# intelligent-environments-lab/CityLearn

Hardware: AMD Instinct MI355X
Metric: building-timesteps/sec at 17 bldgs x 65536 envs; HBM GB/s vs roofline (higher is better)
Workload: dtype f32 (battery soc chain in f64); 1 GPU; citylearn_challenge_2022_phase_all tables (17 buildings, the full year, 8 760 h) x 65536 envs per GPU, cl_step_f32 mode A (one env step per launch, state in HBM, fresh uniform random actions from an 8-tensor ring), env batch sharded over GPUs, no collective; CLD_F64_CHAIN: battery soc chain in float64, degraded capacity carried as the capacity loss; envs_per_gpu=65536, buildings=17, env_pitch=65536, precision=CLD_F64_CHAIN (StepEngine default): 1e-4 free-running over whole episodes, launch=hipGraph replay, reward=RewardFunction, reps=1, statistic=median of reps (each: MAX over ranks)

## Files before the change

### citylearn_amd/csrc/cl_kernels.hip

```cpp
#include "cl_trace.h"
#include "cl_unit.h"
#include "cl_plan.h"
#ifndef CL_LEAN_NT_LOADS
#define CL_LEAN_NT_LOADS true
#endif
#include "cl_philox.h"

#include <type_traits>
#include <mutex>
#include <stdarg.h>
#include <string.h>
#include <stdio.h>

namespace {

int hip_fail(hipError_t e, const char* what) {
    return fail(CL_EHIP, "%s: %s", what, hipGetErrorString(e));
}

hipError_t ensure_dynamic_lds(const void* fn, size_t bytes) {
    struct Seen { const void* fn; int dev; size_t bytes; };
    static Seen seen[64];
    static int n_seen = 0;
    static std::mutex mu;
    int dev = 0;
    if (hipError_t e = hipGetDevice(&dev); e != hipSuccess) return e;
    std::lock_guard<std::mutex> lock(mu);
    for (int i = 0; i < n_seen; ++i)
        if (seen[i].fn == fn && seen[i].dev == dev && seen[i].bytes >= bytes) return hipSuccess;
    if (hipError_t e = hipFuncSetAttribute(fn, hipFuncAttributeMaxDynamicSharedMemorySize, (int)bytes); e != hipSuccess) return e;
    for (int i = 0; i < n_seen; ++i)
        if (seen[i].fn == fn && seen[i].dev == dev) { seen[i].bytes = bytes; return hipSuccess; }
    if (n_seen < 64) seen[n_seen++] = {fn, dev, bytes};
    return hipSuccess;
}

struct StepArgs {
// ... 51 lines not shown
            for (int i = 0; i < VEC; ++i) dst[i] = v[i];
        }
    } else vload<VEC>(dst, p);
}

template <int VEC>
CL_DEV void vstore(float* __restrict__ p, const float (&src)[VEC]) {
    using V = typename Vec<VEC>::type;
    V v;
    if constexpr (VEC == 1) v = src[0];
    else {
#pragma unroll
        for (int i = 0; i < VEC; ++i) v[i] = src[i];
    }
    *reinterpret_cast<V*>(p) = v;
}

template <int VEC, bool NT>
CL_DEV void pstore(float* __restrict__ p, const float (&src)[VEC]) {
    using V = typename Vec<VEC>::type;
    V v;
    if constexpr (VEC == 1) v = src[0];
    else {
#pragma unroll
        for (int i = 0; i < VEC; ++i) v[i] = src[i];
    }
    if constexpr (NT) __builtin_nontemporal_store(v, reinterpret_cast<V*>(p));
    else *reinterpret_cast<V*>(p) = v;
}
struct NtOn { static constexpr bool value = true; };
struct NtOff { static constexpr bool value = false; };

template <int VEC>
CL_DEV void load_action(float (&dst)[VEC], const StepArgs& a, int col, int env0) {
    if (col < 0) {
#pragma unroll
        for (int i = 0; i < VEC; ++i) dst[i] = 0.0f;
        return;
    }
    const float* p = a.actions + (long long)col * a.act_stride_col;
    if (a.act_stride_env == 1) vload<VEC>(dst, p + env0);
    else {
#pragma unroll
        for (int i = 0; i < VEC; ++i) dst[i] = p[(long long)(env0 + i) * a.act_stride_env];
    }
}

#include "cl_flex.h"

constexpr int NQ = CL_NQ;

struct KpiSeries { float prev, ramp, dsum, dmax, msum, mmax, amax; };
CL_DEV void kpi_series_fetch(KpiSeries& s, const float* __restrict__ k, long long n_env);
CL_DEV void kpi_series_apply(float* __restrict__ k, long long n_env, int t, float v, const KpiSeries& s);
CL_DEV void kpi_series_update(float* __restrict__ k, long long n_env, int t, float v);

CL_DEV int fold_shift(int opw) { return opw <= 16 ? 4 : opw <= 32 ? 5 : 6; }
template <int TILE>
CL_DEV float fold_prefetch(const StepArgs& a, int w, int lane, long long plane, int bx, int by) {
    if (a.fused_finish != 2) return 0.0f;
    const int opw = (NQ * TILE + a.n_chunks - 1) / a.n_chunks;
    const int sh = fold_shift(opw);
    const int i = w * 64 + lane, chunk = i >> sh, j = i & ((1 << sh) - 1), o = by * opw + j;
    const int e = bx * TILE + o % TILE;
    if (chunk < a.n_chunks && j < opw && o < NQ * TILE && e < a.n_env)
        return a.out_bldg[(long long)CLO_RESERVED * plane + ((long long)((a.t + 1) & 1) * a.n_chunks + chunk) * NQ * a.n_env + (long long)(o / TILE) * a.n_env + e];
    return 0.0f;
}
CL_DEV void fold_stash(const StepArgs& a, float* lds_fold, int w, int lane, float v) {
    if (a.fused_finish == 2 && w < 16) lds_fold[w * 64 + lane] = v;
}
template <int TILE>
CL_DEV void fold_finish(const StepArgs& a, const float* lds_fold, int w, int lane, int bx, int by) {
    const int opw = (NQ * TILE + a.n_chunks - 1) / a.n_chunks;
    const int sh = fold_shift(opw);
    const int k = lane & 15;
    for (int j = w; j < opw; j += 16) {
        const int o = by * opw + j;
        if (o >= NQ * TILE || bx * TILE + o % TILE >= a.n_env) continue;
// ... 416 lines not shown
                const float rw = cl::unit_reward<false>(rkind, B, S, O.net);
                o_soc[i] = S.soc; o_eff[i] = S.eff; o_deg[i] = S.degcap; o_net[i] = O.net; o_rw[i] = rw;
                q_net[i] += O.net; q_cost[i] += O.cost; q_em[i] += O.emission;
                q_rw[i] += marl_partial ? cl::marl_reward(O.net, 1.0f) : rw;
            }
            if constexpr (FOLD) {
                if (!folded && b + a.nw >= b_hi) { fold_stash(a, lds_fold, w, lane, fold_prev); folded = true; }
            }
            if (b + a.nw < b_hi) fetch(cur, b + a.nw);
            if (batt) {
                pstore<VEC, NT>(a.state + CLS_B_SOC * plane + off, o_soc);
                pstore<VEC, NT>(a.state + CLS_B_EFF * plane + off, o_eff);
                pstore<VEC, NT>(a.state + CLS_B_DEGCAP * plane + off, o_deg);
            }
            pstore<VEC, NT>(a.out_bldg + CLO_NET * plane + off, o_net);
            if (rkind != CLR_MARL) pstore<VEC, NT>(a.out_bldg + CLO_REWARD * plane + off, o_rw);
        }
    }
    if constexpr (FOLD) {
        if (!folded) fold_stash(a, lds_fold, w, lane, fold_prev);
    }
    district_reduce<VEC, false, FOLD>(a, lds, w, lane, env0, live, plane, rkind, q_net, q_cost, q_em, q_rw, a.nw, lds_fold);
}

struct ObsFusedArgs {
    float* __restrict__ obs;
    const float* __restrict__ table;
    int n_cols, pitch, row;
    short start[CL_OBS_FUSED_BLDG + 1];
    cl_obs_dep deps[CLOB_MAX_DEPS];
    int lean_ok;
};

template <int VEC, bool FLEX, bool NT, bool OBS, bool KPI = false, int PREC = 0>
CL_DEV void lean_step_body(const StepArgs& a, float* lds, const ObsFusedArgs* of) {
    constexpr bool F64 = PREC == 1;
    constexpr int TILE = 64 * VEC;
    const int lane = threadIdx.x & 63;
    const int w = __builtin_amdgcn_readfirstlane(threadIdx.x >> 6);
    const int env0 = blockIdx.x * TILE + lane * VEC;
    const bool live = env0 < a.n_env;
    const long long plane = (long long)a.n_bldg * a.ld;
    const int rkind = (a.flags & CLD_REWARD_MASK) >> CLD_REWARD_SHIFT;
    const bool quirk = a.flags & CLD_REF_T0_QUIRK;
    const bool act_by_bldg = (a.flags & CLD_ES_COL_IS_BLDG) && a.act_stride_env == 1;
    const int ts_row = a.t + (a.env_row0 ? a.env_row0[(blockIdx.x * TILE) / CL_ROW0_BLOCK] : 0);
    const int bb[2] = {w, w + a.nw};
    const bool own[2] = {bb[0] < a.n_bldg, bb[1] < a.n_bldg};

    float q_net[VEC], q_cost[VEC], q_em[VEC], q_rw[VEC];
#pragma unroll
    for (int i = 0; i < VEC; ++i) q_net[i] = q_cost[i] = q_em[i] = q_rw[i] = 0.0f;
    float s_soc[2][VEC], s_eff[2][VEC], s_deg[2][VEC], a_es[2][VEC];
    [[maybe_unused]] float s_efl[2][VEC], s_dgl[2][VEC];
    constexpr bool NTL = NT && CL_LEAN_NT_LOADS && (KPI || FLEX || VEC == 2);
    CL_TRACE_DECL;
    CL_TRACE_ENTRY(0);
    CL_TRACE_CYCLES_ENTRY(4);
    if (live) {
#pragma unroll
        for (int m = 0; m < 2; ++m) {
            if (!own[m]) continue;
            const long long off = (long long)bb[m] * a.ld + env0;
            pload<VEC, NTL>(s_soc[m], a.state + CLS_B_SOC * plane + off);
            pload<VEC, NTL>(s_eff[m], a.state + CLS_B_EFF * plane + off);
            pload<VEC, NTL>(s_deg[m], a.state + CLS_B_DEGCAP * plane + off);
            if constexpr (F64) {
                pload<VEC, NTL>(s_efl[m], a.state + CLS_B_EFF_LO * plane + off);
                pload<VEC, NTL>(s_dgl[m], a.state + CLS_B_DEGCAP_LO * plane + off);
            }
            if (act_by_bldg) pload<VEC, NTL>(a_es[m], a.actions + (long long)bb[m] * a.act_stride_col + env0);
        }
    }
#pragma unroll
    for (int m = 0; m < 2; ++m) {
        if (!own[m]) continue;
        const int b = bb[m];
        cl::Bp B;
        cl::load_bp<false>(B, a.params + (long long)b * CL_NP);
        cl::Row R;
        cl::load_row<false>(R, a.ts + ((long long)ts_row * a.n_bldg + b) * CL_NF, B.flags);
        [[maybe_unused]] int od_n = 0, od_col[CL_OBS_FUSED_PER_BLDG], od_src[CL_OBS_FUSED_PER_BLDG];
        [[maybe_unused]] float od_scale[CL_OBS_FUSED_PER_BLDG], od_base[CL_OBS_FUSED_PER_BLDG];
        if constexpr (OBS) {
            const float* __restrict__ trow = of->table + (size_t)(of->row + (ts_row - a.t)) * of->n_cols;
            const int d0 = of->start[b];
            od_n = of->start[b + 1] - d0;
#pragma unroll
            for (int k = 0; k < CL_OBS_FUSED_PER_BLDG; ++k) {
                const int d = min(d0 + min(k, max(od_n - 1, 0)), CLOB_MAX_DEPS - 1);
                od_col[k] = of->deps[d].col; od_src[k] = of->deps[d].src; od_scale[k] = of->deps[d].scale;
                od_base[k] = trow[od_col[k]];
            }
        }
        if (!live) continue;
        const long long off = (long long)b * a.ld + env0;
        const bool batt = B.flags & CLF_BATTERY;
        if (!act_by_bldg) load_action<VEC>(a_es[m], a, B.a_es, env0);
        CL_TRACE_WAITV(1 + 4 * m, s_deg[m][0]);
        float o_net[VEC], o_rw[VEC];
        [[maybe_unused]] float o_cb[VEC];
        const int fbi = (FLEX && (B.flags & CLF_FLEX)) ? (int)B.p[CLP_FLEX_INDEX] : -1;
        float x_load[VEC];
        if (FLEX && fbi >= 0) vload<VEC>(x_load, a.flex_out + (long long)CLX_LOAD * a.n_flex_bldg * a.n_env + (long long)fbi * a.n_env + env0);
        if constexpr (FLEX) {
#pragma unroll
            for (int i = 0; i < VEC; ++i) {
                cl::State S;
                S.soc = batt ? s_soc[m][i] : 0.0f; S.eff = batt ? s_eff[m][i] : 1.0f; S.degcap = batt ? s_deg[m][i] : 0.0f;
                S.cs = S.hs = S.ds = 0.0f;
                const cl::Act act = {0.0f, 0.0f, 0.0f, B.a_es >= 0 ? a_es[m][i] : 0.0f, 0.0f, 0.0f};
                cl::Out O;
                cl::unit_step<false>(B, R, a.t, quirk, act, S, O);
                if (FLEX && fbi >= 0) cl::apply_flex(false, R.price, R.carbon, x_load[i], 0.0f, O);
                const float rw = cl::unit_reward<false>(rkind, B, S, O.net);
                s_soc[m][i] = S.soc; s_eff[m][i] = S.eff; s_deg[m][i] = S.degcap;
                o_net[i] = O.net; o_rw[i] = rw;
                q_net[i] += O.net; q_cost[i] += O.cost; q_em[i] += O.emission;
                q_rw[i] += (FLEX && rkind == CLR_EV) ? cl::marl_reward(O.net, 1.0f) : rw;
            }
        } else {
            const bool first = quirk && a.t == 0;
            float c_ns = first ? 3.0f * R.nsl : R.nsl;
            float sol = R.sol;
            const float cbk = first ? 2.0f : 1.0f;
            CL_PIN_V(c_ns); CL_PIN_V(sol);
            float soc_rw[VEC];
            if (F64 && batt) {
                if constexpr (F64) {
                    cl::BattP64 B64;
                    cl::load_batt64(B64, B.p);
                    if (B.a_es < 0) {
#pragma unroll
                        for (int i = 0; i < VEC; ++i) a_es[m][i] = 0.0f;
                    }
#pragma unroll
                    for (int i = 0; i < VEC; ++i) {
                        cl::State S = {s_soc[m][i], s_eff[m][i], s_deg[m][i], 0.0f, 0.0f, 0.0f, s_efl[m][i], s_dgl[m][i]};
                        const float eb = cl::battery_charge_ref(B64, (double)a_es[m][i] * B64.pow * B64.dt / B64.r, a.t == 0, S);
                        s_soc[m][i] = S.soc; s_eff[m][i] = S.eff; s_deg[m][i] = S.degcap; s_efl[m][i] = S.eff_lo; s_dgl[m][i] = S.deg_lo;
                        soc_rw[i] = S.soc;
                        o_cb[i] = cbk * eb;
                        o_net[i] = fmaf(c_ns + o_cb[i], B.r, sol);
                    }
                }
            } else if (PREC == 2 && batt) {
                if constexpr (PREC == 2) {
                    cl::BattC bc;
                    cl::load_battc(bc, B.p);
                    if (B.a_es < 0) {
#pragma unroll
                        for (int i = 0; i < VEC; ++i) a_es[m][i] = 0.0f;
                    }
#pragma unroll
                    for (int i = 0; i < VEC; ++i) {
                        cl::State S = {s_soc[m][i], s_eff[m][i], s_deg[m][i], 0.0f, 0.0f, 0.0f};
                        const float eb = cl::battery_charge_chain(bc, a_es[m][i], INFINITY, S);
                        s_soc[m][i] = S.soc; s_eff[m][i] = S.eff; s_deg[m][i] = S.degcap;
                        soc_rw[i] = S.soc;
                        o_cb[i] = cbk * eb;
                        o_net[i] = fmaf(c_ns + o_cb[i], B.r, sol);
                    }
                }
            } else if (batt) {
                cl::BattP Bv = B.batt;
                CL_PIN_V(Bv.cpc_a0); CL_PIN_V(Bv.cpc_b0); CL_PIN_V(Bv.cpc_a1); CL_PIN_V(Bv.cpc_b1);
                CL_PIN_V(Bv.pec_a0); CL_PIN_V(Bv.pec_b0); CL_PIN_V(Bv.pec_a1); CL_PIN_V(Bv.pec_b1);
                CL_PIN_V(Bv.pec_a2); CL_PIN_V(Bv.pec_b2); CL_PIN_V(Bv.pec_a3); CL_PIN_V(Bv.pec_b3);
                if (B.a_es < 0) {
#pragma unroll
                    for (int i = 0; i < VEC; ++i) a_es[m][i] = 0.0f;
                }
#pragma unroll
                for (int i = 0; i < VEC; ++i) {
                    cl::State S = {s_soc[m][i], s_eff[m][i], s_deg[m][i], 0.0f, 0.0f, 0.0f};
                    const float eb = cl::battery_energy(Bv, a_es[m][i] * Bv.pdt, S);
                    s_soc[m][i] = S.soc; s_eff[m][i] = S.eff; s_deg[m][i] = S.degcap;
                    soc_rw[i] = S.soc;
                    o_cb[i] = cbk * eb;
                    o_net[i] = fmaf(c_ns + o_cb[i], B.r, sol);
                }
            } else {
#pragma unroll
                for (int i = 0; i < VEC; ++i) { o_net[i] = fmaf(c_ns + 0.0f, B.r, sol); soc_rw[i] = 0.0f; o_cb[i] = 0.0f; }
            }
            cl::lean_rewards<VEC>(rkind, B, soc_rw, o_net, o_rw);
#pragma unroll
            for (int i = 0; i < VEC; ++i) {
                q_net[i] += o_net[i]; q_cost[i] += cl::mul_rn(o_net[i], R.price); q_em[i] += fmaxf(0.0f, o_net[i] * R.carbon);
                q_rw[i] += o_rw[i];
            }
        }
        CL_TRACE_AFTER(2 + 4 * m, o_rw[VEC - 1]);
        if (batt) {
            pstore<VEC, NT>(a.state + CLS_B_SOC * plane + off, s_soc[m]);
            pstore<VEC, NT>(a.state + CLS_B_EFF * plane + off, s_eff[m]);
            pstore<VEC, NT>(a.state + CLS_B_DEGCAP * plane + off, s_deg[m]);
            if constexpr (F64) {
                pstore<VEC, NT>(a.state + CLS_B_EFF_LO * plane + off, s_efl[m]);
                pstore<VEC, NT>(a.state + CLS_B_DEGCAP_LO * plane + off, s_dgl[m]);
            }
        }
        pstore<VEC, NT>(a.out_bldg + CLO_NET * plane + off, o_net);
        if (rkind != CLR_MARL && !(FLEX && rkind == CLR_EV)) pstore<VEC, NT>(a.out_bldg + CLO_REWARD * plane + off, o_rw);
        if constexpr (KPI && !FLEX) {
            float k_pos[VEC], k_net[VEC], k_em[VEC], k_cost[VEC];
            float* kp = a.kpi_bldg + off;
            vload<VEC>(k_pos, kp + (long long)CLK_C_POS * plane); vload<VEC>(k_net, kp + (long long)CLK_C_NET * plane);
            vload<VEC>(k_em, kp + (long long)CLK_C_EMISSION * plane); vload<VEC>(k_cost, kp + (long long)CLK_C_COST * plane);
            const bool block_sums = lane == 0 && (blockIdx.x * TILE) % CL_ROW0_BLOCK == 0;
            float b_pos = 0.0f, b_net = 0.0f, b_em = 0.0f, b_cost = 0.0f, b_exp = 0.0f;
            if (block_sums) {
                b_pos = kp[(long long)CLK_B_POS * plane]; b_net = kp[(long long)CLK_B_NET * plane];
                b_em = kp[(long long)CLK_B_EMISSION * plane]; b_cost = kp[(long long)CLK_B_COST * plane];
                b_exp = kp[(long long)CLK_EXPECTED_ALL * plane];
            }
#pragma unroll
            for (int i = 0; i < VEC; ++i) {
                k_pos[i] += fmaxf(o_net[i], 0.0f); k_net[i] += o_net[i];
                k_em[i] += fmaxf(o_net[i] * R.carbon, 0.0f); k_cost[i] += fmaxf(o_net[i] * R.price, 0.0f);
            }
            pstore<VEC, NT>(kp + (long long)CLK_C_POS * plane, k_pos); pstore<VEC, NT>(kp + (long long)CLK_C_NET * plane, k_net);
            pstore<VEC, NT>(kp + (long long)CLK_C_EMISSION * plane, k_em); pstore<VEC, NT>(kp + (long long)CLK_C_COST * plane, k_cost);
            const float c_ns0 = (quirk && a.t == 0) ? 3.0f * R.nsl : R.nsl;
            const float base = fmaf(c_ns0, B.r, R.sol);
            if (lane == 0) lds[(size_t)a.nw * NQ * TILE + b] = base;
            if (block_sums) {
                kp[(long long)CLK_B_POS * plane] = b_pos + fmaxf(base, 0.0f);
                kp[(long long)CLK_B_NET * plane] = b_net + base;
                kp[(long long)CLK_B_EMISSION * plane] = b_em + fmaxf(base * R.carbon, 0.0f);
                kp[(long long)CLK_B_COST * plane] = b_cost + fmaxf(base * R.price, 0.0f);
                kp[(long long)CLK_EXPECTED_ALL * plane] = b_exp + R.nsl;
            }
        }
        if constexpr (OBS) {
            float* tile = lds + (size_t)a.nw * NQ * TILE;
#pragma unroll
            for (int k = 0; k < CL_OBS_FUSED_PER_BLDG; ++k) {
                if (k >= od_n) break;
                const int col = od_col[k], src = od_src[k];
                const float scale = od_scale[k], base = od_base[k];
                const bool is_out = (src >> 28) == CLOB_KIND_OUT;
                const int pl = (src >> 20) & 0xFF;
#pragma unroll
                for (int i = 0; i < VEC; ++i) {
                    const float v = is_out ? (pl == CLO_NET ? o_net[i] : o_rw[i])
                                           : (pl == CLS_B_SOC ? s_soc[m][i] : pl == CLS_B_EFF ? s_eff[m][i] : s_deg[m][i]);
                    tile[(size_t)(lane * VEC + i) * of->pitch + col] = fmaf(v, scale, base);
                }
            }
        }
        CL_TRACE_AFTER(3 + 4 * m, q_rw[0]);
    }
    if constexpr (OBS) {
        if (w == 0) {
            float* tile = lds + (size_t)a.nw * NQ * TILE;
            for (int c = of->n_cols; c < of->pitch; ++c) {
#pragma unroll
                for (int i = 0; i < VEC; ++i) tile[(size_t)(lane * VEC + i) * of->pitch + c] = 0.0f;
            }
        }
    }
    CL_TRACE_AFTER(13, q_net[0]);
    [[maybe_unused]] KpiSeries base_pre;
    [[maybe_unused]] const bool base_writer = KPI && !FLEX && threadIdx.x == blockDim.x - 1 && (blockIdx.x * TILE) % CL_ROW0_BLOCK == 0;
    if constexpr (KPI && !FLEX) {
        if (base_writer) kpi_series_fetch(base_pre, a.kpi_env + (long long)CLKE_PER_COND * a.n_env + blockIdx.x * TILE, a.n_env);
    }
    district_reduce<VEC, FLEX, false, KPI && !FLEX>(a, lds, w, lane, env0, live, plane, rkind, q_net, q_cost, q_em, q_rw, a.nw);
    if constexpr (KPI && !FLEX) {
        if (base_writer) {
            float sum = 0.0f;
            for (int b = 0; b < a.n_bldg; ++b) sum += lds[(size_t)a.nw * NQ * TILE + b];
            kpi_series_apply(a.kpi_env + (long long)CLKE_PER_COND * a.n_env + blockIdx.x * TILE, a.n_env, a.t, sum, base_pre);
        }
    }
    if constexpr (OBS) {
        typedef float f4 __attribute__((ext_vector_type(4)));
        const int tile_env0 = blockIdx.x * TILE;
        const int rows = min(TILE, a.n_env - tile_env0);
        const f4* src4 = reinterpret_cast<const f4*>(lds + (size_t)a.nw * NQ * TILE);
        f4* dst4 = reinterpret_cast<f4*>(of->obs + (size_t)tile_env0 * of->pitch);
        const int total4 = rows * of->pitch / 4;
        for (int q = threadIdx.x; q < total4; q += blockDim.x) {
            if constexpr (NT) __builtin_nontemporal_store(src4[q], dst4 + q);
            else dst4[q] = src4[q];
        }
    }
    CL_TRACE_FLUSH();
}

template <int VEC, bool FLEX, bool NT>
__global__ void __launch_bounds__(1024) cl_step_lean_kernel(const StepArgs a) {
    extern __shared__ __attribute__((aligned(16))) float lds[];
    lean_step_body<VEC, FLEX, NT, false>(a, lds, nullptr);
}

template <int VEC, bool NT>
__global__ void __launch_bounds__(1024) cl_step_lean_f64_kernel(const StepArgs a) {
    extern __shared__ __attribute__((aligned(16))) float lds[];
    lean_step_body<VEC, false, NT, false, false, 1>(a, lds, nullptr);
}

template <int VEC, bool NT>
__global__ void __launch_bounds__(1024) cl_step_lean_chain_kernel(const StepArgs a) {
    extern __shared__ __attribute__((aligned(16))) float lds[];
    lean_step_body<VEC, false, NT, false, false, 2>(a, lds, nullptr);
}

template <int VEC, bool NT>
__global__ void __launch_bounds__(1024) cl_step_lean_kpi_chain_kernel(const StepArgs a) {
    extern __shared__ __attribute__((aligned(16))) float lds[];
    lean_step_body<VEC, false, NT, false, true, 2>(a, lds, nullptr);
}

template <int VEC, bool NT>
__global__ void __launch_bounds__(1024) cl_step_lean_obs_chain_kernel(const StepArgs a, const ObsFusedArgs of) {
    extern __shared__ __attribute__((aligned(16))) float lds[];
    lean_step_body<VEC, false, NT, true, false, 2>(a, lds, &of);
}

template <int VEC, bool NT>
__global__ void __launch_bounds__(1024) cl_step_lean_kpi_kernel(const StepArgs a) {
    extern __shared__ __attribute__((aligned(16))) float lds[];
    lean_step_body<VEC, false, NT, false, true>(a, lds, nullptr);
}

template <int VEC, bool NT>
__global__ void __launch_bounds__(1024) cl_step_lean_obs_kernel(const StepArgs a, const ObsFusedArgs of) {
    extern __shared__ __attribute__((aligned(16))) float lds[];
    lean_step_body<VEC, false, NT, true>(a, lds, &of);
}

template <int NB, bool NT, int VEC = 1, int PREC = 0>
__global__ void __launch_bounds__(256 / VEC) cl_step_envmajor_kernel(const StepArgs a) {
    constexpr int THREADS = 256 / VEC, TILE = 256;
    const int env = blockIdx.x * TILE + threadIdx.x * VEC;
    const bool live = env < a.n_env;
    const long long plane = (long long)a.n_bldg * a.ld;
    const int rkind = (a.flags & CLD_REWARD_MASK) >> CLD_REWARD_SHIFT;
// ... 1126 lines not shown
```

### citylearn_amd/abi.py

```python
from __future__ import annotations

import re
from pathlib import Path

HEADER = Path(__file__).resolve().parent.parent / 'include' / 'citylearn_amd.h'


def _strip_comments(text: str) -> str:
    text = re.sub(r'/\*.*?\*/', ' ', text, flags=re.S)
    return re.sub(r'//[^\n]*', ' ', text)


def _parse(text: str) -> dict:
    text = _strip_comments(text)
    out: dict = {}
    for m in re.finditer(r'#define\s+(CL\w+)\s+(.+)', text):
        name, expr = m.group(1), m.group(2).strip()
        expr = re.sub(r'(0x[0-9a-fA-F]+|\d+)[uU]\b', r'\1', expr)
        try:
            out[name] = int(eval(expr, {'__builtins__': {}}, out))
        except Exception:
            pass
    for m in re.finditer(r'enum\s+(\w+)\s*\{(.*?)\}', text, flags=re.S):
        nxt = 0
        for item in m.group(2).split(','):
            item = item.strip()
            if not item:
                continue
            if '=' in item:
                name, val = [s.strip() for s in item.split('=')]
                nxt = int(eval(val, {'__builtins__': {}}, out))
            else:
                name = item
            out[name] = nxt
            nxt += 1
    return out


_C = _parse(HEADER.read_text())
globals().update(_C)
CONSTANTS = dict(_C)

EXPORTED_SYMBOLS = sorted(set(re.findall(r'\b(cl_\w+)\s*\(', _strip_comments(HEADER.read_text()))))

assert _C['CLP_USED'] <= _C['CLP_F_FIRST'] and _C['CLP_F_LAST'] < _C['CLP_D_FIRST'] and _C['CLP_D_LAST'] < _C['CL_NP'], 'cl_param overflows CL_NP'
assert _C['CLPD_USED'] * 2 <= _C['CLP_D_LAST'] - _C['CLP_D_FIRST'] + 1 and _C['CLP_D_FIRST'] % 2 == 0 and _C['CL_NP'] % 2 == 0
assert _C['CLP_D_LAST'] < _C['CLP_C_FIRST'] and _C['CLP_C_LAST'] < _C['CL_NP'] and _C['CLP_C_FIRST'] % 2 == 0 and _C['CLPC_USED'] * 2 <= _C['CLP_C_LAST'] - _C['CLP_C_FIRST'] + 1
```

### citylearn_amd/csrc/cl_unit.h

```cpp
#pragma once

#include <stdint.h>
#include "../../include/citylearn_amd.h"

#ifdef CL_HOST_SHIM
#include <math.h>
#include <string.h>
#define CL_DEV inline
namespace cl {
inline float rcp(float x) { return 1.0f / x; }
inline float rsq(float x) { return 1.0f / sqrtf(x); }
inline float fsqrt(float x) { return sqrtf(x); }
inline float med3(float a, float b, float c) { return fmaxf(fminf(a, b), fminf(fmaxf(a, b), c)); }
inline float __uint_as_float(uint32_t u) { float f; memcpy(&f, &u, 4); return f; }
inline float __powf(float a, float b) { return powf(a, b); }
}
#else
#include <hip/hip_runtime.h>
#define CL_DEV __device__ __forceinline__
namespace cl {
CL_DEV float rcp(float x) { return __builtin_amdgcn_rcpf(x); }
CL_DEV float rsq(float x) { return __builtin_amdgcn_rsqf(x); }
CL_DEV float fsqrt(float x) { return __builtin_amdgcn_sqrtf(x); }
CL_DEV float med3(float a, float b, float c) { return __builtin_amdgcn_fmed3f(a, b, c); }
// ... 496 lines not shown
}

template <int N>
CL_DEV void lean_rewards(int kind, const Bp& B, const float (&soc)[N], const float (&net)[N], float (&rw)[N]) {
    switch (kind) {
    case CLR_INDEPENDENT_SAC:
#pragma unroll
        for (int i = 0; i < N; ++i) rw[i] = fminf(-net[i], 0.0f);
        break;
    case CLR_SOLAR_PENALTY: {
        const bool has = pw(B.p, CLP_L_CAP) > CL_ZDP;
#pragma unroll
        for (int i = 0; i < N; ++i) {
            const float sg = net[i] > 0.0f ? 1.0f : (net[i] < 0.0f ? -1.0f : 0.0f), an = fabsf(net[i]);
            rw[i] = has ? -(1.0f + sg * soc[i]) * an : 0.0f;
        }
        break;
    }
    case CLR_MARL: case CLR_EV:
#pragma unroll
        for (int i = 0; i < N; ++i) rw[i] = net[i];
        break;
    default:
        if (B.rw_exponent == 1.0f) {
#pragma unroll
            for (int i = 0; i < N; ++i) rw[i] = -fmaxf(net[i], 0.0f);
        } else {
#pragma unroll
            for (int i = 0; i < N; ++i) rw[i] = -__powf(fmaxf(net[i], 0.0f), B.rw_exponent);
        }
    }
}

CL_DEV float marl_reward(float net, float district_net) {
    const float sg = net < 0.0f ? 1.0f : (net > 0.0f ? -1.0f : 0.0f);
    return sg * 0.01f * net * net * fmaxf(0.0f, district_net);
}

}
```

### citylearn_amd/schema.py

```python
from __future__ import annotations

import hashlib
import json
import math
import os
from dataclasses import dataclass, field
from pathlib import Path
from typing import Any, Dict, List, Mapping, Optional, Sequence, Tuple, Union

import numpy as np

from . import abi

ZERO_DIVISION_PLACEHOLDER = 1e-6
TOLERANCE = 1e-4
DEFAULT_COMFORT_BAND = 2.0

_STORAGE_ACTIONS = ('cooling_storage', 'heating_storage', 'dhw_storage', 'electrical_storage')
_DEVICE_ACTIONS = ('cooling_device', 'heating_device', 'cooling_or_heating_device')
_ACTION_SLOT = {
    'cooling_storage': abi.CLP_ACT_COOL_STO, 'heating_storage': abi.CLP_ACT_HEAT_STO,
    'dhw_storage': abi.CLP_ACT_DHW_STO, 'electrical_storage': abi.CLP_ACT_ELEC_STO,
    'cooling_device': abi.CLP_ACT_COOL_DEV, 'heating_device': abi.CLP_ACT_HEAT_DEV,
    'cooling_or_heating_device': abi.CLP_ACT_COH_DEV,
# ... 537 lines not shown
                c64[abi.CLPC_PEC_X1 + 2 * (k - 1)], c64[abi.CLPC_PEC_DB1 + 2 * (k - 1)] = ex[k], eslope[k] - eslope[k - 1]
            chain_ok = (np.all(np.diff(cx) > 0) and np.all(np.diff(ex) > 0) and cx[2] >= 1.0 and ex[4] >= 1.0 and np.max(cy) <= 1.0
                        and np.all(np.isfinite(c64[:abi.CLPC_VALID])))
            c64[abi.CLPC_VALID] = 1.0 if chain_ok else 0.0
            for tank, base in ((b.cooling_storage, abi.CLP_CS_IRTE), (b.heating_storage, abi.CLP_HS_IRTE),
                               (b.dhw_storage, abi.CLP_DS_IRTE)):
                pf[i, base + 0] = 1.0 / math.sqrt(tank.efficiency)
                pf[i, base + 1] = 1.0 / max(float(tank.capacity), ZERO_DIVISION_PLACEHOLDER)
                pf[i, base + 2] = float(tank.capacity) * (1.0 - tank.loss_coefficient * r)
            s = b.series
            w = slice(start, end + 1)
            t_out = s['outdoor_dry_bulb_temperature'][w]
            ts[:, i, abi.CLT_NSL] = s['non_shiftable_load'][w]
            ts[:, i, abi.CLT_SOLAR] = -(b.pv_nominal_power * np.array(s['solar_generation'][w]) / 1000.0)
            ts[:, i, abi.CLT_COOL_DEM] = s['cooling_demand'][w]
            ts[:, i, abi.CLT_HEAT_DEM] = s['heating_demand'][w]
            ts[:, i, abi.CLT_DHW_DEM] = s['dhw_demand'][w]
            ts[:, i, abi.CLT_COP_COOL] = cd.cop(t_out, heating=False)
            ts[:, i, abi.CLT_COP_HEAT] = hd.cop(t_out, heating=True) if hd.is_heat_pump else hd.efficiency
            ts[:, i, abi.CLT_COP_DHW] = dd.cop(t_out, heating=True) if dd.is_heat_pump else dd.efficiency
            ts[:, i, abi.CLT_PRICE] = s['electricity_pricing'][w]
            ts[:, i, abi.CLT_CARBON] = s['carbon_intensity'][w]
            outage[:, i] = self.outage_signal(b, start, end)
            ts[:, i, abi.CLT_OUTAGE] = outage[:, i] if b.outage.simulate else 0.0
            ts[:, i, abi.CLT_HVAC_MODE] = s['hvac_mode'][w]
            ts[:, i, abi.CLT_T_OUT] = t_out
            pf[i, abi.CLP_T0_HEAT_DIV] = ts[0, i, abi.CLT_COP_HEAT] if hd.is_heat_pump else dd.efficiency
            pf[i, abi.CLP_T0_IHEAT_DIV] = 1.0 / float(pf[i, abi.CLP_T0_HEAT_DIV])
            with np.errstate(divide='ignore'):
                for c_col, i_col in ((abi.CLT_COP_COOL, abi.CLT_ICOP_COOL), (abi.CLT_COP_HEAT, abi.CLT_ICOP_HEAT),
                                     (abi.CLT_COP_DHW, abi.CLT_ICOP_DHW)):
                    ts[:, i, i_col] = 1.0 / ts[:, i, c_col].astype(np.float64)
        _pack_full_block(params)
        from .flex import pack_flex
        flex = pack_flex(self, start, T, aligned=window is not None)
        return EpisodeTables(params=params, ts=ts, start=start, end=end, outage=outage, flex=flex)


def _pack_full_block(params: np.ndarray):
    pf = params.view(np.float32)
    F = abi.CLP_F_FIRST
    params[:, abi.CLP_F_FLAGS] = params[:, abi.CLP_FLAGS]
    params[:, abi.CLP_F_ACT:abi.CLP_F_ACT + 7] = params[:, [abi.CLP_ACT_COOL_STO, abi.CLP_ACT_HEAT_STO, abi.CLP_ACT_DHW_STO, abi.CLP_ACT_ELEC_STO,
                                                           abi.CLP_ACT_COOL_DEV, abi.CLP_ACT_HEAT_DEV, abi.CLP_ACT_COH_DEV]]
    params[:, abi.CLP_F_HEAD:abi.CLP_F_HEAD + 8] = params[:, [abi.CLP_DT_HOURS, abi.CLP_L_TSR, abi.CLP_CD_POW, abi.CLP_HD_POW, abi.CLP_DD_POW,
                                                             abi.CLP_T0_IHEAT_DIV, abi.CLP_DYN_WARMUP, abi.CLP_L_RW_EXPONENT]]
    dt = pf[:, abi.CLP_DT_HOURS]
    scales = (pf[:, abi.CLP_CS_CAP], pf[:, abi.CLP_CS_CAP] * dt, pf[:, abi.CLP_HS_CAP] * dt)
    for k, (raw, der) in enumerate(((abi.CLP_CS_CAP, abi.CLP_CS_IRTE), (abi.CLP_HS_CAP, abi.CLP_HS_IRTE), (abi.CLP_DS_CAP, abi.CLP_DS_IRTE))):
        base = abi.CLP_F_TANK + 8 * k
        params[:, base:base + 7] = params[:, [raw, der + 2, raw + 2, der, der + 1, raw + 4, raw + 5]]
        pf[:, base + 7] = scales[k].astype(np.float32)
    params[:, abi.CLP_F_BATT:abi.CLP_F_BATT + 24] = params[:, abi.CLP_L_PDT:abi.CLP_L_PDT + 24]
    assert abi.CLP_L_PDT + 23 == abi.CLP_L_PEC_B3 and F + 63 == abi.CLP_F_LAST



def _read_csv(path: str) -> Dict[str, np.ndarray]:
    import pandas as pd
    frame = pd.read_csv(path)
    return {c: frame[c].to_numpy() for c in frame.columns}


class _Noise:

    def __init__(self, std: float, generator=None):
        self.std = float(std or 0.0)
        self.generator = np.random if generator is None else generator

    def __call__(self, like) -> np.ndarray:
        shape = np.asarray(like).shape
        return np.zeros(shape) if self.std <= 0 else self.generator.normal(loc=0, scale=self.std, size=shape)


def _energy_simulation_series(cols: Mapping[str, np.ndarray], seconds_per_time_step: float, noise: _Noise = _Noise(0.0)) -> Tuple[Dict[str, np.ndarray], float]:
    for k in _ES_REQUIRED:
        if k not in cols:
            raise KeyError(f'energy_simulation file lacks column {k!r}')
    n = len(cols['solar_generation'])
    f32 = lambda k, default=0.0: (np.zeros(n, dtype='float32') + default) if k not in cols else np.array(cols[k], dtype='float32')
    out: Dict[str, np.ndarray] = {}
    for k in ('month', 'hour', 'day_type'):
        out[k] = np.array(cols[k], dtype='int32')
    out['indoor_dry_bulb_temperature'] = np.clip(np.array(cols['indoor_dry_bulb_temperature'], dtype='float32') + noise(cols['indoor_dry_bulb_temperature']), -90, 57)
    out['solar_generation'] = np.array(cols['solar_generation'], dtype='float32') + noise(cols['indoor_dry_bulb_temperature'])
    for k in ('non_shiftable_load', 'dhw_demand', 'cooling_demand', 'heating_demand'):
        out[k] = np.array(cols[k], dtype='float32')
# ... 426 lines not shown
```

### include/citylearn_amd.h

```cpp
#ifndef CITYLEARN_AMD_H
#define CITYLEARN_AMD_H

#include <stdint.h>

#ifdef __cplusplus
extern "C" {
#endif

#define CL_ABI_VERSION 9

#define CL_OK            0
#define CL_EINVAL       -1
#define CL_ENULL        -2
#define CL_EALIGN       -3
#define CL_EHIP         -4
#define CL_ERANGE       -5

#define CL_NP  320
#define CL_NF   16
#define CL_NS    8
#define CL_NO   18
#define CL_NQ    4
#define CL_NKB  12
#define CL_NKE  24
// ... 22 lines not shown
    CLP_L_ACT_ES,
    CLP_L_TSR,
    CLP_L_PDT,
    CLP_L_POW,
    CLP_L_CAP,
    CLP_L_CAPL,
    CLP_L_INV_CAP,
    CLP_L_INV_POW,
    CLP_L_OMD,
    CLP_L_DEGK,
    CLP_L_CPC_X1,
    CLP_L_CPC_A0, CLP_L_CPC_B0, CLP_L_CPC_A1, CLP_L_CPC_B1,
    CLP_L_PEC_X1, CLP_L_PEC_X2, CLP_L_PEC_X3,
    CLP_L_PEC_A0, CLP_L_PEC_B0, CLP_L_PEC_A1, CLP_L_PEC_B1, CLP_L_PEC_A2, CLP_L_PEC_B2, CLP_L_PEC_A3, CLP_L_PEC_B3,
    CLP_L_RW_EXPONENT,
    CLP_L_SOC0, CLP_L_EFF0,
    CLP_L_LAST = CLP_L_EFF0,
    CLP_CS_IRTE, CLP_CS_ICAP, CLP_CS_CAPL,
    CLP_HS_IRTE, CLP_HS_ICAP, CLP_HS_CAPL,
    CLP_DS_IRTE, CLP_DS_ICAP, CLP_DS_CAPL,
    CLP_T0_IHEAT_DIV,
    CLP_FLEX_INDEX,
    CLP_USED,
    CLP_F_FIRST = 128,
    CLP_F_FLAGS = CLP_F_FIRST,
    CLP_F_ACT = CLP_F_FIRST + 1,
    CLP_F_HEAD = CLP_F_FIRST + 8,
    CLP_F_TANK = CLP_F_FIRST + 16,
    CLP_F_BATT = CLP_F_FIRST + 40,
    CLP_F_LAST = CLP_F_FIRST + 63,
    CLP_D_FIRST = 192,
    CLP_D_LAST = CLP_D_FIRST + 63,
    CLP_C_FIRST = 256,
    CLP_C_LAST = CLP_C_FIRST + 63
};
enum cl_param_chain {
    CLPC_CAP = 0,
    CLPC_OML,
    CLPC_RCAP,
    CLPC_PDT,
    CLPC_POW, CLPC_RPOW,
    CLPC_TSR,
    CLPC_CPC_A0, CLPC_CPC_B0, CLPC_CPC_X1, CLPC_CPC_DB1,
    CLPC_PEC_A0, CLPC_PEC_B0, CLPC_PEC_X1, CLPC_PEC_DB1, CLPC_PEC_X2, CLPC_PEC_DB2, CLPC_PEC_X3, CLPC_PEC_DB3,
    CLPC_VALID,
    CLPC_USED
};
enum cl_param_f64 {
    CLPD_TSR = 0,
    CLPD_DT,
    CLPD_POW, CLPD_CAP,
    CLPD_OML,
    CLPD_SOC_LIMIT,
    CLPD_CLCCAP,
    CLPD_EFF0,
    CLPD_CPC_X0, CLPD_CPC_X1, CLPD_CPC_X2, CLPD_CPC_Y0, CLPD_CPC_Y1, CLPD_CPC_Y2,
    CLPD_PEC_X0, CLPD_PEC_X1, CLPD_PEC_X2, CLPD_PEC_X3, CLPD_PEC_X4,
    CLPD_PEC_Y0, CLPD_PEC_Y1, CLPD_PEC_Y2, CLPD_PEC_Y3, CLPD_PEC_Y4,
    CLPD_RCAP,
    CLPD_RPOW,
    CLPD_RCPC_01, CLPD_RCPC_12,
    CLPD_RPEC_01, CLPD_RPEC_12, CLPD_RPEC_23, CLPD_RPEC_34,
    CLPD_USED
};

#define CLF_BATTERY      (1u << 0)
// ... 299 lines not shown
```

Before: 145.9 billion building-timesteps/s.

## Prefetch second building's params and row via lanes into LDS stash

For the lean PREC==2, VEC==4 path, each lane fetches one word of the second building's parameters, time-series fields and battery coefficients early, before the state loads, then parks them in the wave's LDS reduction row. The second building later reads its params from LDS instead of issuing scalar loads after the first building's work. This aims to hide the latency of the second building's uniform loads behind the first building's computation, at the cost of extra LDS traffic, wave barriers and more complex control flow. The early path is only taken when the grid has at most 480 blocks; otherwise the fetch happens inline.

```diff
diff --git a/citylearn_amd/csrc/cl_kernels.hip b/citylearn_amd/csrc/cl_kernels.hip
--- a/citylearn_amd/csrc/cl_kernels.hip
+++ b/citylearn_amd/csrc/cl_kernels.hip
@@ -3,6 +3,9 @@
 #include "cl_plan.h"
 #ifndef CL_LEAN_NT_LOADS
 #define CL_LEAN_NT_LOADS true
+#endif
+#ifndef CL_LEAN_LDS_STASH
+#define CL_LEAN_LDS_STASH true
 #endif
 #include "cl_philox.h"
 
@@ -637,9 +640,33 @@
     float s_soc[2][VEC], s_eff[2][VEC], s_deg[2][VEC], a_es[2][VEC];
     [[maybe_unused]] float s_efl[2][VEC], s_dgl[2][VEC];
     constexpr bool NTL = NT && CL_LEAN_NT_LOADS && (KPI || FLEX || VEC == 2);
+    constexpr bool STASH = CL_LEAN_LDS_STASH && !FLEX && !OBS && !KPI && PREC == 2 && VEC == 4;
+    const bool early = STASH && own[1] && gridDim.x <= 480;
+    constexpr int PW = CLP_L_LAST - CLP_L_FIRST + 1, CW = PREC == 2 ? 2 * CLPC_USED : 0, SW = PW + 4 + CW;
+    static_assert(PW + 4 <= 64 && SW <= 128 && SW <= NQ * 64, "the stash: at most two words per lane, inside the wave's reduction row");
+    uint32_t* const sp = reinterpret_cast<uint32_t*>(lds) + (size_t)w * NQ * TILE;
+    [[maybe_unused]] uint32_t st0 = 0u, st1 = 0u;
     CL_TRACE_DECL;
     CL_TRACE_ENTRY(0);
     CL_TRACE_CYCLES_ENTRY(4);
+    auto fetch_second = [&] {
+        const uint32_t* __restrict__ p1 = a.params + (long long)bb[1] * CL_NP;
+        const uint32_t* __restrict__ q1 = reinterpret_cast<const uint32_t*>(a.ts + ((long long)ts_row * a.n_bldg + bb[1]) * CL_NF);
+        const int kr = lane - PW;
+        const uint32_t* src = lane < PW ? p1 + CLP_L_FIRST + lane
+                            : kr < 4 ? q1 + (kr == 0 ? CLT_NSL : kr == 1 ? CLT_SOLAR : kr == 2 ? CLT_PRICE : CLT_CARBON)
+                            : p1 + CLP_C_FIRST + (kr - 4);
+        st0 = *src;
+        if (lane + 64 < SW) st1 = p1[CLP_C_FIRST + (lane + 64 - PW - 4)];
+    };
+    auto park_second = [&] {
+        sp[lane] = st0;
+        if (lane + 64 < SW) sp[lane + 64] = st1;
+        __builtin_amdgcn_wave_barrier();
+    };
+    if constexpr (STASH) {
+        if (early) fetch_second();
+    }
     if (live) {
 #pragma unroll
         for (int m = 0; m < 2; ++m) {
@@ -660,9 +687,26 @@
         if (!own[m]) continue;
         const int b = bb[m];
         cl::Bp B;
-        cl::load_bp<false>(B, a.params + (long long)b * CL_NP);
         cl::Row R;
-        cl::load_row<false>(R, a.ts + ((long long)ts_row * a.n_bldg + b) * CL_NF, B.flags);
+        [[maybe_unused]] cl::BattC bc;
+        if (STASH && m == 1) {
+            if constexpr (STASH) {
+                if (!early) { fetch_second(); park_second(); }
+                cl::load_bp<false>(B, sp - CLP_L_FIRST);
+                B.flags = __builtin_amdgcn_readfirstlane(B.flags); B.a_es = __builtin_amdgcn_readfirstlane(B.a_es);
+                R.nsl = __uint_as_float(sp[PW]); R.sol = __uint_as_float(sp[PW + 1]);
+                R.price = __uint_as_float(sp[PW + 2]); R.carbon = __uint_as_float(sp[PW + 3]);
+                R.outage = false;
+                cl::load_battc64(bc, sp + (PW + 4) - CLP_C_FIRST);
+                bc.cap32 = B.batt.cap; bc.omd32 = B.batt.omd; bc.degk = B.batt.degk;
+            }
+        } else {
+            cl::load_bp<false>(B, a.params + (long long)b * CL_NP);
+            cl::load_row<false>(R, a.ts + ((long long)ts_row * a.n_bldg + b) * CL_NF, B.flags);
+        }
+        if constexpr (STASH) {
+            if (m == 0 && early) park_second();
+        }
         [[maybe_unused]] int od_n = 0, od_col[CL_OBS_FUSED_PER_BLDG], od_src[CL_OBS_FUSED_PER_BLDG];
         [[maybe_unused]] float od_scale[CL_OBS_FUSED_PER_BLDG], od_base[CL_OBS_FUSED_PER_BLDG];
         if constexpr (OBS) {
@@ -679,8 +723,15 @@
         if (!live) continue;
         const long long off = (long long)b * a.ld + env0;
         const bool batt = B.flags & CLF_BATTERY;
-        if (!act_by_bldg) load_action<VEC>(a_es[m], a, B.a_es, env0);
-        CL_TRACE_WAITV(1 + 4 * m, s_deg[m][0]);
+        if (!act_by_bldg) {
+            load_action<VEC>(a_es[m], a, B.a_es, env0);
+            if (STASH && m == 1) {
+#pragma unroll
+                for (int i = 0; i < VEC; ++i) CL_PIN_V(a_es[m][i]);
+            }
+        }
+        if (STASH && m == 1) CL_TRACE_AFTER(1 + 4 * m, R.nsl);
+        else CL_TRACE_WAITV(1 + 4 * m, s_deg[m][0]);
         float o_net[VEC], o_rw[VEC];
         [[maybe_unused]] float o_cb[VEC];
         const int fbi = (FLEX && (B.flags & CLF_FLEX)) ? (int)B.p[CLP_FLEX_INDEX] : -1;
@@ -729,8 +780,7 @@
                 }
             } else if (PREC == 2 && batt) {
                 if constexpr (PREC == 2) {
-                    cl::BattC bc;
-                    cl::load_battc(bc, B.p);
+                    if (!(STASH && m == 1)) cl::load_battc(bc, B.p);
                     if (B.a_es < 0) {
 #pragma unroll
                         for (int i = 0; i < VEC; ++i) a_es[m][i] = 0.0f;
```

Result: slower. 141.5 billion building-timesteps/s (-3.1%).

## Burst-load per-building chain constants as scalar loads and prefetch second building

Applied to the files above, without the earlier changes.

For the f64-chain lean step kernel, per-building parameters and timestep row values are packed into a contiguous mirror block in the param array. They are fetched through constant-address-space (scalar) loads in a burst, with the second building's block prefetched while the first building's battery chain runs. State stores move earlier, right after the battery update, and the kernel is specialised on the default reward kind. This aims to cut scattered load latency and serialisation between the two buildings each wave handles, at the cost of more SGPR/VGPR pressure and inline-asm pinning that could hurt scheduling.

```diff
diff --git a/citylearn_amd/abi.py b/citylearn_amd/abi.py
--- a/citylearn_amd/abi.py
+++ b/citylearn_amd/abi.py
@@ -46,3 +46,4 @@
 assert _C['CLP_USED'] <= _C['CLP_F_FIRST'] and _C['CLP_F_LAST'] < _C['CLP_D_FIRST'] and _C['CLP_D_LAST'] < _C['CL_NP'], 'cl_param overflows CL_NP'
 assert _C['CLPD_USED'] * 2 <= _C['CLP_D_LAST'] - _C['CLP_D_FIRST'] + 1 and _C['CLP_D_FIRST'] % 2 == 0 and _C['CL_NP'] % 2 == 0
 assert _C['CLP_D_LAST'] < _C['CLP_C_FIRST'] and _C['CLP_C_LAST'] < _C['CL_NP'] and _C['CLP_C_FIRST'] % 2 == 0 and _C['CLPC_USED'] * 2 <= _C['CLP_C_LAST'] - _C['CLP_C_FIRST'] + 1
+assert _C['CLP_C_FIRST'] + _C['CLPC_USED'] * 2 <= _C['CLP_CM_FIRST'] and _C['CLP_CM_LAST'] <= _C['CLP_C_LAST'] and _C['CLP_CM_FIRST'] % 8 == 0
diff --git a/citylearn_amd/csrc/cl_kernels.hip b/citylearn_amd/csrc/cl_kernels.hip
--- a/citylearn_amd/csrc/cl_kernels.hip
+++ b/citylearn_amd/csrc/cl_kernels.hip
@@ -120,19 +120,21 @@
 struct NtOff { static constexpr bool value = false; };
 
 template <int VEC>
-CL_DEV void load_action(float (&dst)[VEC], const StepArgs& a, int col, int env0) {
+CL_DEV void load_action(float (&dst)[VEC], const StepArgs& a, int col, int env0, long long stride_env) {
     if (col < 0) {
 #pragma unroll
         for (int i = 0; i < VEC; ++i) dst[i] = 0.0f;
         return;
     }
     const float* p = a.actions + (long long)col * a.act_stride_col;
-    if (a.act_stride_env == 1) vload<VEC>(dst, p + env0);
+    if (stride_env == 1) vload<VEC>(dst, p + env0);
     else {
 #pragma unroll
-        for (int i = 0; i < VEC; ++i) dst[i] = p[(long long)(env0 + i) * a.act_stride_env];
-    }
-}
+        for (int i = 0; i < VEC; ++i) dst[i] = p[(long long)(env0 + i) * stride_env];
+    }
+}
+template <int VEC>
+CL_DEV void load_action(float (&dst)[VEC], const StepArgs& a, int col, int env0) { load_action<VEC>(dst, a, col, env0, a.act_stride_env); }
 
 #include "cl_flex.h"
 
@@ -615,16 +617,63 @@
     int lean_ok;
 };
 
-template <int VEC, bool FLEX, bool NT, bool OBS, bool KPI = false, int PREC = 0>
+typedef const uint32_t __attribute__((address_space(4)))* cl_ku32;
+struct ChainBlk {
+    uint32_t flags; int a_es;
+    float nsl, sol, price, carbon;
+    float r, rw_exponent;
+    cl::BattC bc;
+};
+CL_DEV float kw(cl_ku32 p, int slot) { return __uint_as_float(p[slot]); }
+CL_DEV double kd(cl_ku32 p, int k) {
+    const uint64_t bits = (uint64_t)p[CLP_C_FIRST + 2 * k] | ((uint64_t)p[CLP_C_FIRST + 2 * k + 1] << 32);
+    double d;
+    __builtin_memcpy(&d, &bits, 8);
+    return d;
+}
+CL_DEV void chain_blk_load_a(ChainBlk& K, cl_ku32 p, cl_ku32 q) {
+    K.flags = p[CLP_CM_FLAGS]; K.a_es = (int)p[CLP_CM_ACT_ES];
+    K.nsl = kw(q, CLT_NSL); K.sol = kw(q, CLT_SOLAR); K.price = kw(q, CLT_PRICE); K.carbon = kw(q, CLT_CARBON);
+    cl::BattC& C = K.bc;
+    C.cap = kd(p, CLPC_CAP); C.oml = kd(p, CLPC_OML); C.rcap = kd(p, CLPC_RCAP); C.pdt = kd(p, CLPC_PDT); C.pow = kd(p, CLPC_POW);
+    C.rpow = kd(p, CLPC_RPOW); C.r = kd(p, CLPC_TSR);
+    C.ca0 = kd(p, CLPC_CPC_A0); C.cb0 = kd(p, CLPC_CPC_B0); C.cx1 = kd(p, CLPC_CPC_X1); C.cdb1 = kd(p, CLPC_CPC_DB1);
+    C.cap32 = kw(p, CLP_CM_CAP); C.omd32 = kw(p, CLP_CM_OMD); C.degk = kw(p, CLP_CM_DEGK);
+    K.r = kw(p, CLP_CM_TSR); K.rw_exponent = kw(p, CLP_CM_RW_EXPONENT);
+}
+CL_DEV void chain_blk_load_b(ChainBlk& K, cl_ku32 p) {
+    cl::BattC& C = K.bc;
+    C.ea0 = kd(p, CLPC_PEC_A0); C.eb0 = kd(p, CLPC_PEC_B0); C.ex1 = kd(p, CLPC_PEC_X1); C.edb1 = kd(p, CLPC_PEC_DB1);
+    C.ex2 = kd(p, CLPC_PEC_X2); C.edb2 = kd(p, CLPC_PEC_DB2); C.ex3 = kd(p, CLPC_PEC_X3); C.edb3 = kd(p, CLPC_PEC_DB3);
+}
+CL_DEV void chain_blk_load(ChainBlk& K, const uint32_t* __restrict__ params, const float* __restrict__ row) {
+    const cl_ku32 p = (cl_ku32)params, q = (cl_ku32)reinterpret_cast<const uint32_t*>(row);
+    chain_blk_load_a(K, p, q);
+    chain_blk_load_b(K, p);
+}
+#define CL_CHAIN_BLK_LAND(K, ...) \
+    asm("" : "+s"((K).flags), "+s"((K).a_es), "+s"((K).nsl), "+s"((K).sol), "+s"((K).price), "+s"((K).carbon), "+s"((K).r), "+s"((K).rw_exponent), \
+             "+s"((K).bc.cap32), "+s"((K).bc.omd32), "+s"((K).bc.degk), "+s"((K).bc.cap), \
+             "+v"((K).bc.oml), "+v"((K).bc.rcap), "+v"((K).bc.pdt), "+v"((K).bc.pow), "+v"((K).bc.rpow), "+v"((K).bc.r), \
+             "+v"((K).bc.ca0), "+v"((K).bc.cb0), "+v"((K).bc.cx1), "+v"((K).bc.cdb1) __VA_ARGS__)
+CL_DEV void chain_blk_load_2(ChainBlk& K, const uint32_t* __restrict__ params, const float* __restrict__ row) {
+    cl_ku32 p = (cl_ku32)params;
+    chain_blk_load_a(K, p, (cl_ku32)reinterpret_cast<const uint32_t*>(row));
+    CL_CHAIN_BLK_LAND(K, , "+s"(p));
+    chain_blk_load_b(K, p);
+}
+
+template <int VEC, bool FLEX, bool NT, bool OBS, bool KPI = false, int PREC = 0, int RK = -1>
 CL_DEV void lean_step_body(const StepArgs& a, float* lds, const ObsFusedArgs* of) {
     constexpr bool F64 = PREC == 1;
+    constexpr bool BURST = PREC == 2 && !OBS && !KPI;
     constexpr int TILE = 64 * VEC;
     const int lane = threadIdx.x & 63;
     const int w = __builtin_amdgcn_readfirstlane(threadIdx.x >> 6);
     const int env0 = blockIdx.x * TILE + lane * VEC;
     const bool live = env0 < a.n_env;
     const long long plane = (long long)a.n_bldg * a.ld;
-    const int rkind = (a.flags & CLD_REWARD_MASK) >> CLD_REWARD_SHIFT;
+    const int rkind = RK >= 0 ? RK : (int)((a.flags & CLD_REWARD_MASK) >> CLD_REWARD_SHIFT);
     const bool quirk = a.flags & CLD_REF_T0_QUIRK;
     const bool act_by_bldg = (a.flags & CLD_ES_COL_IS_BLDG) && a.act_stride_env == 1;
     const int ts_row = a.t + (a.env_row0 ? a.env_row0[(blockIdx.x * TILE) / CL_ROW0_BLOCK] : 0);
@@ -655,14 +704,32 @@
             if (act_by_bldg) pload<VEC, NTL>(a_es[m], a.actions + (long long)bb[m] * a.act_stride_col + env0);
         }
     }
-#pragma unroll
-    for (int m = 0; m < 2; ++m) {
-        if (!own[m]) continue;
+    [[maybe_unused]] ChainBlk K[2];
+    [[maybe_unused]] int by_bldg = 0;
+    if constexpr (BURST) by_bldg = __builtin_amdgcn_readfirstlane((int)act_by_bldg);
+    [[maybe_unused]] auto fetch_second = [&]() __attribute__((always_inline)) {
+        const int b1 = own[1] ? bb[1] : bb[0];
+        chain_blk_load(K[1], a.params + (long long)b1 * CL_NP, a.ts + ((long long)ts_row * a.n_bldg + b1) * CL_NF);
+    };
+    auto turn = [&](auto mc) __attribute__((always_inline)) {
+        constexpr int m = decltype(mc)::value;
+        if (!own[m]) return;
         const int b = bb[m];
+        if constexpr (BURST) {
+            if (m == 0) chain_blk_load_2(K[0], a.params + (long long)b * CL_NP, a.ts + ((long long)ts_row * a.n_bldg + b) * CL_NF);
+        }
         cl::Bp B;
-        cl::load_bp<false>(B, a.params + (long long)b * CL_NP);
         cl::Row R;
-        cl::load_row<false>(R, a.ts + ((long long)ts_row * a.n_bldg + b) * CL_NF, B.flags);
+        if constexpr (BURST) {
+            if (!live) return;
+            if (m == 1) CL_CHAIN_BLK_LAND(K[1]);
+            B.p = a.params + (long long)b * CL_NP;
+            B.flags = K[m].flags; B.a_es = K[m].a_es; B.r = K[m].r; B.rw_exponent = K[m].rw_exponent;
+            R.nsl = K[m].nsl; R.sol = K[m].sol; R.price = K[m].price; R.carbon = K[m].carbon;
+        } else {
+            cl::load_bp<false>(B, a.params + (long long)b * CL_NP);
+            cl::load_row<false>(R, a.ts + ((long long)ts_row * a.n_bldg + b) * CL_NF, B.flags);
+        }
         [[maybe_unused]] int od_n = 0, od_col[CL_OBS_FUSED_PER_BLDG], od_src[CL_OBS_FUSED_PER_BLDG];
         [[maybe_unused]] float od_scale[CL_OBS_FUSED_PER_BLDG], od_base[CL_OBS_FUSED_PER_BLDG];
         if constexpr (OBS) {
@@ -676,10 +743,31 @@
                 od_base[k] = trow[od_col[k]];
             }
         }
-        if (!live) continue;
+        if (!live) return;
         const long long off = (long long)b * a.ld + env0;
         const bool batt = B.flags & CLF_BATTERY;
-        if (!act_by_bldg) load_action<VEC>(a_es[m], a, B.a_es, env0);
+        bool act_here = act_by_bldg;
+        if constexpr (BURST) {
+            int by_bldg_here = __builtin_amdgcn_readfirstlane(by_bldg);
+            asm("" : "+s"(by_bldg_here) : "n"(m));
+            act_here = by_bldg_here != 0;
+        }
+        if (!act_here) {
+            long long stride_env = a.act_stride_env;
+            if constexpr (BURST) asm("" : "+s"(stride_env) : "n"(m));
+            load_action<VEC>(a_es[m], a, B.a_es, env0, stride_env);
+            if constexpr (BURST) {
+#pragma unroll
+                for (int i = 0; i < VEC; ++i) CL_PIN_V(a_es[m][i]);
+            }
+        } else if constexpr (BURST) {
+#pragma unroll
+            for (int i = 0; i < VEC; ++i) CL_PIN_V(a_es[m][i]);
+        }
+        if constexpr (BURST) {
+#pragma unroll
+            for (int i = 0; i < VEC; ++i) { CL_PIN_V(s_soc[m][i]); CL_PIN_V(s_eff[m][i]); CL_PIN_V(s_deg[m][i]); }
+        }
         CL_TRACE_WAITV(1 + 4 * m, s_deg[m][0]);
         float o_net[VEC], o_rw[VEC];
         [[maybe_unused]] float o_cb[VEC];
@@ -730,7 +818,10 @@
             } else if (PREC == 2 && batt) {
                 if constexpr (PREC == 2) {
                     cl::BattC bc;
-                    cl::load_battc(bc, B.p);
+                    if constexpr (BURST) {
+                        bc = K[m].bc;
+                        CL_PIN_V(bc.ea0); CL_PIN_V(bc.eb0); CL_PIN_V(bc.ex1); CL_PIN_V(bc.edb1); CL_PIN_V(bc.ex2); CL_PIN_V(bc.edb2); CL_PIN_V(bc.ex3); CL_PIN_V(bc.edb3);
+                    } else cl::load_battc(bc, B.p);
                     if (B.a_es < 0) {
 #pragma unroll
                         for (int i = 0; i < VEC; ++i) a_es[m][i] = 0.0f;
@@ -743,6 +834,12 @@
                         soc_rw[i] = S.soc;
                         o_cb[i] = cbk * eb;
                         o_net[i] = fmaf(c_ns + o_cb[i], B.r, sol);
+                    }
+                    if constexpr (BURST) {
+                        pstore<VEC, NT>(a.state + CLS_B_SOC * plane + off, s_soc[m]);
+                        pstore<VEC, NT>(a.state + CLS_B_EFF * plane + off, s_eff[m]);
+                        pstore<VEC, NT>(a.state + CLS_B_DEGCAP * plane + off, s_deg[m]);
+                        if (m == 0) fetch_second();
                     }
                 }
             } else if (batt) {
@@ -766,8 +863,12 @@
             } else {
 #pragma unroll
                 for (int i = 0; i < VEC; ++i) { o_net[i] = fmaf(c_ns + 0.0f, B.r, sol); soc_rw[i] = 0.0f; o_cb[i] = 0.0f; }
-            }
-            cl::lean_rewards<VEC>(rkind, B, soc_rw, o_net, o_rw);
+                if constexpr (BURST) {
+                    if (m == 0) fetch_second();
+                }
+            }
+            if constexpr (BURST) cl::lean_rewards_v<VEC>(rkind, K[m].bc.cap32, B.rw_exponent, soc_rw, o_net, o_rw);
+            else cl::lean_rewards<VEC>(rkind, B, soc_rw, o_net, o_rw);
 #pragma unroll
             for (int i = 0; i < VEC; ++i) {
                 q_net[i] += o_net[i]; q_cost[i] += cl::mul_rn(o_net[i], R.price); q_em[i] += fmaxf(0.0f, o_net[i] * R.carbon);
@@ -775,7 +876,7 @@
             }
         }
         CL_TRACE_AFTER(2 + 4 * m, o_rw[VEC - 1]);
-        if (batt) {
+        if (!BURST && batt) {
             pstore<VEC, NT>(a.state + CLS_B_SOC * plane + off, s_soc[m]);
             pstore<VEC, NT>(a.state + CLS_B_EFF * plane + off, s_eff[m]);
             pstore<VEC, NT>(a.state + CLS_B_DEGCAP * plane + off, s_deg[m]);
@@ -785,7 +886,13 @@
             }
         }
         pstore<VEC, NT>(a.out_bldg + CLO_NET * plane + off, o_net);
-        if (rkind != CLR_MARL && !(FLEX && rkind == CLR_EV)) pstore<VEC, NT>(a.out_bldg + CLO_REWARD * plane + off, o_rw);
+        bool store_rw = rkind != CLR_MARL && !(FLEX && rkind == CLR_EV);
+        if constexpr (BURST && RK < 0) {
+            int kind_here = rkind;
+            asm("" : "+s"(kind_here));
+            store_rw = kind_here != CLR_MARL;
+        }
+        if (store_rw) pstore<VEC, NT>(a.out_bldg + CLO_REWARD * plane + off, o_rw);
         if constexpr (KPI && !FLEX) {
             float k_pos[VEC], k_net[VEC], k_em[VEC], k_cost[VEC];
             float* kp = a.kpi_bldg + off;
@@ -834,6 +941,15 @@
             }
         }
         CL_TRACE_AFTER(3 + 4 * m, q_rw[0]);
+    };
+    if constexpr (BURST) {
+        if (own[0] && live) {
+            turn(std::integral_constant<int, 0>{});
+            if (own[1]) turn(std::integral_constant<int, 1>{});
+        }
+    } else {
+        turn(std::integral_constant<int, 0>{});
+        turn(std::integral_constant<int, 1>{});
     }
     if constexpr (OBS) {
         if (w == 0) {
@@ -888,7 +1004,8 @@
 template <int VEC, bool NT>
 __global__ void __launch_bounds__(1024) cl_step_lean_chain_kernel(const StepArgs a) {
     extern __shared__ __attribute__((aligned(16))) float lds[];
-    lean_step_body<VEC, false, NT, false, false, 2>(a, lds, nullptr);
+    if (((a.flags & CLD_REWARD_MASK) >> CLD_REWARD_SHIFT) == CLR_DEFAULT) lean_step_body<VEC, false, NT, false, false, 2, CLR_DEFAULT>(a, lds, nullptr);
+    else lean_step_body<VEC, false, NT, false, false, 2>(a, lds, nullptr);
 }
 
 template <int VEC, bool NT>
diff --git a/citylearn_amd/csrc/cl_unit.h b/citylearn_amd/csrc/cl_unit.h
--- a/citylearn_amd/csrc/cl_unit.h
+++ b/citylearn_amd/csrc/cl_unit.h
@@ -552,6 +552,37 @@
     }
 }
 
+template <int N>
+CL_DEV void lean_rewards_v(int kind, float cap, float exponent, const float (&soc)[N], const float (&net)[N], float (&rw)[N]) {
+    switch (kind) {
+    case CLR_INDEPENDENT_SAC:
+#pragma unroll
+        for (int i = 0; i < N; ++i) rw[i] = fminf(-net[i], 0.0f);
+        break;
+    case CLR_SOLAR_PENALTY: {
+        const bool has = cap > CL_ZDP;
+#pragma unroll
+        for (int i = 0; i < N; ++i) {
+            const float sg = net[i] > 0.0f ? 1.0f : (net[i] < 0.0f ? -1.0f : 0.0f), an = fabsf(net[i]);
+            rw[i] = has ? -(1.0f + sg * soc[i]) * an : 0.0f;
+        }
+        break;
+    }
+    case CLR_MARL: case CLR_EV:
+#pragma unroll
+        for (int i = 0; i < N; ++i) rw[i] = net[i];
+        break;
+    default:
+        if (exponent == 1.0f) {
+#pragma unroll
+            for (int i = 0; i < N; ++i) rw[i] = -fmaxf(net[i], 0.0f);
+        } else {
+#pragma unroll
+            for (int i = 0; i < N; ++i) rw[i] = -__powf(fmaxf(net[i], 0.0f), exponent);
+        }
+    }
+}
+
 CL_DEV float marl_reward(float net, float district_net) {
     const float sg = net < 0.0f ? 1.0f : (net > 0.0f ? -1.0f : 0.0f);
     return sg * 0.01f * net * net * fmaxf(0.0f, district_net);
diff --git a/citylearn_amd/schema.py b/citylearn_amd/schema.py
--- a/citylearn_amd/schema.py
+++ b/citylearn_amd/schema.py
@@ -593,6 +593,7 @@
                                      (abi.CLT_COP_DHW, abi.CLT_ICOP_DHW)):
                     ts[:, i, i_col] = 1.0 / ts[:, i, c_col].astype(np.float64)
         _pack_full_block(params)
+        _pack_chain_mirror(params)
         from .flex import pack_flex
         flex = pack_flex(self, start, T, aligned=window is not None)
         return EpisodeTables(params=params, ts=ts, start=start, end=end, outage=outage, flex=flex)
@@ -614,6 +615,12 @@
         pf[:, base + 7] = scales[k].astype(np.float32)
     params[:, abi.CLP_F_BATT:abi.CLP_F_BATT + 24] = params[:, abi.CLP_L_PDT:abi.CLP_L_PDT + 24]
     assert abi.CLP_L_PDT + 23 == abi.CLP_L_PEC_B3 and F + 63 == abi.CLP_F_LAST
+
+
+def _pack_chain_mirror(params: np.ndarray):
+    src = [abi.CLP_L_FLAGS, abi.CLP_L_ACT_ES, abi.CLP_L_CAP, abi.CLP_L_OMD, abi.CLP_L_DEGK, abi.CLP_L_TSR, abi.CLP_L_RW_EXPONENT]
+    assert abi.CLP_CM_LAST - abi.CLP_CM_FIRST + 1 == len(src)
+    params[:, abi.CLP_CM_FIRST:abi.CLP_CM_LAST + 1] = params[:, src]
 
 
 
diff --git a/include/citylearn_amd.h b/include/citylearn_amd.h
--- a/include/citylearn_amd.h
+++ b/include/citylearn_amd.h
@@ -78,6 +78,13 @@
     CLP_D_FIRST = 192,
     CLP_D_LAST = CLP_D_FIRST + 63,
     CLP_C_FIRST = 256,
+    CLP_CM_FIRST = CLP_C_FIRST + 40,
+    CLP_CM_FLAGS = CLP_CM_FIRST,
+    CLP_CM_ACT_ES,
+    CLP_CM_CAP, CLP_CM_OMD, CLP_CM_DEGK,
+    CLP_CM_TSR,
+    CLP_CM_RW_EXPONENT,
+    CLP_CM_LAST = CLP_CM_RW_EXPONENT,
     CLP_C_LAST = CLP_C_FIRST + 63
 };
 enum cl_param_chain {
```

Measured after the change: 145.8 billion building-timesteps/s before, 144.3 billion building-timesteps/s after. 0.989x the previous value.
